# p768lwy3/torecsys

Measured on AMD Instinct MI355X. Metric: CTR samples/sec fwd+bwd (DeepFM, 39 fields x dim 64), higher is better.
Workload: dtype bf16; 1 GPU; BASELINE.json configs[1]: DeepFM 39 Criteo-shaped fields, MLP [400,400,400], 1000000 total rows, embed_dim 64, batch 65536, uniform indices, uniform field sizes; global_batch=65536, rows=1000000, parallelism=single, microbatches=1, optimizer=none, hipgraph=True, hipgraph_input_sets=1, hipgraph_steps_per_replay=4, fused_lookup_fm=True

## Files before the change

### include/trs_abi.h

```cpp
#ifndef TRS_ABI_H_
#define TRS_ABI_H_

#include <stddef.h>
#include <stdint.h>

#ifdef __cplusplus
extern "C" {
#endif

#define TRS_ABI_VERSION 3

enum { TRS_F32 = 0, TRS_BF16 = 1 };
enum { TRS_I64 = 0, TRS_I32 = 1 };
enum {
  TRS_OK = 0,
  TRS_EINVAL = -1,
  TRS_EDTYPE = -2,
  TRS_ESHAPE = -3,
  TRS_EALIGN = -4,
  TRS_ELAUNCH = -5,
  TRS_EWORKSPACE = -6
};

typedef void* trs_stream_t;
// ... 184 lines not shown
int trs_rowdot_fwd(const void* h, const void* w, const void* bias, int64_t rows, int32_t C, int32_t dtype, void* out,
                   trs_stream_t stream);
size_t trs_rowdot_bwd_workspace_bytes(int64_t rows, int32_t C);
int trs_rowdot_bwd(const void* g, const void* h, const void* w, int64_t rows, int32_t C, int32_t dtype, void* gh,
                   float* gw, float* gb, void* workspace, size_t ws_bytes, trs_stream_t stream);

int trs_transpose_pad(const void* in, int64_t B, int32_t R, int32_t Cc, int32_t ld_in, void* out, int32_t ld_out,
                      int32_t dtype, trs_stream_t stream);

int trs_cat_head_fwd(const void* a, const void* d, const void* w, const void* bias, int64_t rows, int32_t N, int32_t Ea,
                     int32_t Eb, int32_t dtype, void* out, trs_stream_t stream);
size_t trs_cat_head_bwd_workspace_bytes(int64_t rows, int32_t N, int32_t Ea, int32_t Eb);
int trs_cat_head_bwd(const void* g, const void* a, const void* d, const void* w, int64_t rows, int32_t N, int32_t Ea,
                     int32_t Eb, int32_t dtype, void* ga, void* gd, float* gw, float* gb, void* workspace,
                     size_t ws_bytes, trs_stream_t stream);

int trs_wgrad_finish(const float* part, int32_t S, int32_t R, int32_t Cc, int32_t out_rows, int32_t out_cols,
                     int32_t dtype, void* gw, const float* gb_f32, void* gb, trs_stream_t stream);
int trs_wgrad_finish_t(const float* part, int32_t S, int32_t Cc, int32_t R, int32_t out_rows, int32_t out_cols,
                       int32_t dtype, void* gw, const float* gb_f32, void* gb, trs_stream_t stream);
int32_t trs_wgrad_rows_splits(int32_t M, int32_t N, int64_t rows);
int trs_wgrad_rows(const void* g, int32_t ldg, const void* x, int32_t ldx, int64_t rows, int32_t M, int32_t N,
                   int32_t dtype, int32_t S, float* part, trs_stream_t stream);
int32_t trs_wgrad_wide_splits(int32_t M_x, int32_t N_g, int32_t ld_g, int64_t rows);
int trs_wgrad_wide(const void* x, int32_t ldx, const void* g, int32_t ldg, int64_t rows, int32_t M_x, int32_t N_g,
                   int32_t S, float* part, trs_stream_t stream);
int trs_copy_padded_many(const int64_t* desc, int32_t n, int32_t elem_size, int64_t max_elems, trs_stream_t stream);

int32_t trs_cin_glue_blocks(int64_t B);
int trs_cin_glue_stats(const void* y, int64_t B, int32_t E, int32_t C, int32_t dtype, float* partial,
                       trs_stream_t stream);
int trs_cin_glue_fwd(const void* y, const float* scale, const float* shift, int64_t B, int32_t E, int32_t C, int32_t D,
                     int32_t Hs, int32_t dtype, void* hidden, void* pooled, trs_stream_t stream);
int trs_cin_glue_bwd_reduce(const void* y, const void* g_hidden, const void* g_pooled, const float* scale,
                            const float* shift, const float* mean, const float* invstd, int64_t B, int32_t E, int32_t C,
                            int32_t D, int32_t Hs, int32_t dtype, float* partial, trs_stream_t stream);
int trs_cin_glue_bwd_apply(const void* y, const void* g_hidden, const void* g_pooled, const float* scale,
                           const float* shift, const float* mean, const float* invstd, const float* c1, const float* c2,
                           int64_t B, int32_t E, int32_t C, int32_t D, int32_t Hs, int32_t dtype, void* gy,
                           trs_stream_t stream);
int trs_cin_glue_cf_supported(int32_t E, int32_t C);
int trs_cin_glue_fwd_cf(const void* y, const float* scale, const float* shift, int64_t B, int32_t E, int32_t C,
                        int32_t D, int32_t Hs, int32_t dtype, void* hidden, void* hidden_cf, void* pooled,
                        trs_stream_t stream);
int trs_cin_glue_bwd_apply_cf(const void* y, const void* g_hidden, const void* g_pooled, const float* scale,
                              const float* shift, const float* mean, const float* invstd, const float* c1,
// ... 124 lines not shown
```

### torecsys_amd/_abi.py

```python
from __future__ import annotations

import ctypes
import os
import threading
from ctypes import c_char_p, c_int32, c_int64, c_size_t, c_void_p

import torch

_HERE = os.path.dirname(os.path.abspath(__file__))
LIB_PATH = os.environ.get("TRS_LIB_PATH") or os.path.join(_HERE, "libtrs_hip.so")

TRS_F32, TRS_BF16 = 0, 1
TRS_I64, TRS_I32 = 0, 1

_P, _I32, _I64, _SZ, _F32 = c_void_p, c_int32, c_int64, c_size_t, ctypes.c_float

_OPTIMIZER_TAIL = [_I32, _F32, _P, _F32, _F32, _F32, _P, _P, _P, _SZ, _P]

SIGNATURES = {
    "trs_version": (c_int32, []),
    "trs_last_error_string": (c_char_p, []),
    "trs_rowdot_fwd": (c_int32, [_P, _P, _P, _I64, _I32, _I32, _P, _P]),
    "trs_rowdot_bwd_workspace_bytes": (_SZ, [_I64, _I32]),
    "trs_rowdot_bwd": (c_int32, [_P, _P, _P, _I64, _I32, _I32, _P, _P, _P, _P, _SZ, _P]),
    "trs_transpose_pad": (c_int32, [_P, _I64, _I32, _I32, _I32, _P, _I32, _I32, _P]),
    "trs_cat_head_fwd": (c_int32, [_P, _P, _P, _P, _I64, _I32, _I32, _I32, _I32, _P, _P]),
    "trs_cat_head_bwd_workspace_bytes": (_SZ, [_I64, _I32, _I32, _I32]),
    "trs_cat_head_bwd": (c_int32, [_P, _P, _P, _P, _I64, _I32, _I32, _I32, _I32, _P, _P, _P, _P, _P, _SZ, _P]),
    "trs_wgrad_finish": (c_int32, [_P, _I32, _I32, _I32, _I32, _I32, _I32, _P, _P, _P, _P]),
    "trs_wgrad_finish_t": (c_int32, [_P, _I32, _I32, _I32, _I32, _I32, _I32, _P, _P, _P, _P]),
    "trs_wgrad_rows_splits": (c_int32, [_I32, _I32, _I64]),
    "trs_wgrad_rows": (c_int32, [_P, _I32, _P, _I32, _I64, _I32, _I32, _I32, _I32, _P, _P]),
    "trs_wgrad_wide_splits": (c_int32, [_I32, _I32, _I32, _I64]),
    "trs_wgrad_wide": (c_int32, [_P, _I32, _P, _I32, _I64, _I32, _I32, _I32, _P, _P]),
    "trs_copy_padded_many": (c_int32, [_P, _I32, _I32, _I64, _P]),
    "trs_cin_glue_blocks": (c_int32, [_I64]),
    "trs_cin_glue_stats": (c_int32, [_P, _I64, _I32, _I32, _I32, _P, _P]),
    "trs_cin_glue_fwd": (c_int32, [_P, _P, _P, _I64, _I32, _I32, _I32, _I32, _I32, _P, _P, _P]),
    "trs_cin_glue_bwd_reduce": (c_int32, [_P, _P, _P, _P, _P, _P, _P, _I64, _I32, _I32, _I32, _I32, _I32, _P, _P]),
    "trs_cin_glue_bwd_apply": (c_int32, [_P, _P, _P, _P, _P, _P, _P, _P, _P, _I64, _I32, _I32, _I32, _I32, _I32, _P, _P]),
    "trs_cin_glue_cf_supported": (c_int32, [_I32, _I32]),
    "trs_cin_glue_fwd_cf": (c_int32, [_P, _P, _P, _I64, _I32, _I32, _I32, _I32, _I32, _P, _P, _P, _P]),
    "trs_cin_glue_bwd_apply_cf": (c_int32, [_P, _P, _P, _P, _P, _P, _P, _P, _P, _I64, _I32, _I32, _I32, _I32, _I32, _P, _P, _P,
                                            _P]),
    "trs_opn_vec_fwd": (c_int32, [_P, _P, _I32, _I64, _I32, _I32, _I32, _P, _P]),
    "trs_opn_vec_bwd_workspace_bytes": (_SZ, [_I64, _I32, _I32]),
    "trs_opn_vec_bwd": (c_int32, [_P, _P, _P, _I32, _I64, _I32, _I32, _I32, _P, _P, _P, _SZ, _P]),
    "trs_pair_mul_fwd": (c_int32, [_P, _P, _P, _I32, _I64, _I32, _I32, _I32, _P, _P]),
    "trs_rows_mul_bias_fwd": (c_int32, [_P, _P, _P, _I32, _I64, _I32, _I32, _I32, _P, _P]),
    "trs_rows_mul_bwd": (c_int32, [_P, _P, _P, _I64, _I32, _I32, _P, _P, _P]),
    "trs_pair_mul_bwd": (c_int32, [_P, _P, _P, _I64, _I32, _I32, _I32, _P, _P, _P]),
    "trs_pair_bilinear_fwd": (c_int32, [_P, _P, _I32, _P, _I32, _I32, _I64, _I32, _I32, _I32, _P, _P]),
    "trs_pair_bilinear_bwd_data": (c_int32, [_P, _P, _P, _I32, _I32, _I64, _I32, _I32, _I32, _P, _P, _P]),
    "trs_pair_bilinear_fwd_mfma": (c_int32, [_P, _P, _P, _P, _I32, _I32, _I64, _I32, _I32, _I32, _P, _P]),
    "trs_pair_bilinear_bwd_data_mfma": (c_int32, [_P, _P, _P, _P, _P, _I32, _P, _P, _I32, _P, _I32, _I64, _I32, _I32, _I32,
# ... 319 lines not shown
```

### torecsys_amd/csrc/mlp_epilogue.hip

```cpp
#include <algorithm>

#include "trs_common.hpp"

namespace trs {

constexpr int RB_THREADS = 256;

template <typename T>
__global__ __launch_bounds__(RB_THREADS) void relu_bwd_bias_kernel(const uint4* __restrict__ gy, const uint4* __restrict__ y,
                                                                   uint4* __restrict__ gz, float* __restrict__ part,
                                                                   int64_t rows, int vpr ,
                                                                   int rows_per_band) {
  constexpr int VE = Vec16<T>::VE;
  __shared__ float red[RB_THREADS][VE];
  const int64_t r0 = (int64_t)blockIdx.x * rows_per_band;
  const int64_t r1 = r0 + rows_per_band < rows ? r0 + rows_per_band : rows;
  const int cv = threadIdx.x % vpr, rl = threadIdx.x / vpr, rstep = RB_THREADS / vpr;
  float acc[VE];
#pragma unroll
  for (int k = 0; k < VE; ++k) acc[k] = 0.f;
  if (rl < rstep) {
    constexpr int U = 4;
    for (int64_t rb = r0 + rl; rb < r1; rb += (int64_t)rstep * U) {
      uint4 gv[U], yv[U];
// ... 188 lines not shown

__global__ void rowdot_finish_kernel(const float* __restrict__ tmp, int C, float* __restrict__ gw,
                                         float* __restrict__ gb) {
  const int c = blockIdx.x * blockDim.x + threadIdx.x;
  if (c < C) gw[c] = tmp[c];
  else if (c == C) gb[0] = tmp[C];
}

static int rowdot_fwd_blocks(int64_t rows, int lpr) {
  const int rpp = 256 / lpr;
  return (int)std::min<int64_t>((rows + (int64_t)rpp * 4 - 1) / ((int64_t)rpp * 4), 8192);
}
static int rowdot_blocks(int64_t rows, int lpr) {
  const int rpp = 256 / lpr;
  return (int)std::min<int64_t>((rows + rpp - 1) / rpp, 1023);
}
static bool rowdot_shape_ok(int C, int dtype) {
  const int ve = dtype == TRS_F32 ? 4 : 8;
  const int lpr = C % ve == 0 ? C / ve : 0;
  return lpr >= 1 && lpr <= 64 && (lpr & (lpr - 1)) == 0;
}

template <typename T>
__global__ __launch_bounds__(256) void wgrad_finish_kernel(const float* __restrict__ part, int S, int R, int Cc,
                                                          int out_rows, int out_cols, T* __restrict__ gw,
                                                          const float* __restrict__ gbf, T* __restrict__ gb) {
  const int c = blockIdx.x * 256 + threadIdx.x;
  if ((int)blockIdx.y == out_rows) {
    if (gb != nullptr && c < out_rows) gb[c] = from_f32<T>(gbf[c]);
    return;
  }
  if (c >= out_cols) return;
  const int r = blockIdx.y;
  const float* p = part + (size_t)r * Cc + c;
  const size_t stride = (size_t)R * Cc;
  float a0 = 0.f, a1 = 0.f, a2 = 0.f, a3 = 0.f;
  int s = 0;
  for (; s + 4 <= S; s += 4) {
    a0 += p[(size_t)s * stride];
    a1 += p[(size_t)(s + 1) * stride];
    a2 += p[(size_t)(s + 2) * stride];
    a3 += p[(size_t)(s + 3) * stride];
  }
  for (; s < S; ++s) a0 += p[(size_t)s * stride];
  gw[(size_t)r * out_cols + c] = from_f32<T>((a0 + a1) + (a2 + a3));
}

constexpr int WF_SL = 16;
constexpr int WF_COLS = 256 / WF_SL;
template <typename T>
__global__ __launch_bounds__(256) void wgrad_finish_few_rows_kernel(const float* __restrict__ part, int S, int R, int Cc,
                                                                   int out_rows, int out_cols, T* __restrict__ gw,
                                                                   const float* __restrict__ gbf, T* __restrict__ gb) {
  __shared__ float red[WF_SL][WF_COLS + 1];
  if ((int)blockIdx.y == out_rows) {
    const int c = blockIdx.x * 256 + threadIdx.x;
    if (gb != nullptr && c < out_rows) gb[c] = from_f32<T>(gbf[c]);
    return;
  }
  const int cl = threadIdx.x % WF_COLS, sl = threadIdx.x / WF_COLS;
  const int c = blockIdx.x * WF_COLS + cl;
  const int r = blockIdx.y;
  const size_t stride = (size_t)R * Cc;
  float a0 = 0.f, a1 = 0.f, a2 = 0.f, a3 = 0.f;
  if (c < out_cols) {
    const float* p = part + (size_t)r * Cc + c;
    int s = sl;
    for (; s + 3 * WF_SL < S; s += 4 * WF_SL) {
// ... 382 lines not shown
  TRS_REQUIRE(gb == nullptr || out_rows <= ((out_cols + 255) / 256) * 256, TRS_ESHAPE,
              "wgrad_finish: out_rows %d exceeds the bias row of workgroups", out_rows);
  hipStream_t s = (hipStream_t)stream;
  dim3 grid((out_cols + 255) / 256, out_rows + 1);
  if (S >= 4 * WF_SL && (int64_t)grid.x * out_rows < 64) {
    dim3 gridf((out_cols + WF_COLS - 1) / WF_COLS, out_rows + 1);
    if (dtype == TRS_F32)
      hipLaunchKernelGGL((wgrad_finish_few_rows_kernel<float>), gridf, dim3(256), 0, s, part, S, R, Cc, out_rows, out_cols,
                         (float*)gw, gb_f32, (float*)gb);
    else
      hipLaunchKernelGGL((wgrad_finish_few_rows_kernel<bf16_t>), gridf, dim3(256), 0, s, part, S, R, Cc, out_rows, out_cols,
                         (bf16_t*)gw, gb_f32, (bf16_t*)gb);
    return check_launch("wgrad_finish");
  }
  if (dtype == TRS_F32)
    hipLaunchKernelGGL((wgrad_finish_kernel<float>), grid, dim3(256), 0, s, part, S, R, Cc, out_rows, out_cols,
                       (float*)gw, gb_f32, (float*)gb);
  else
    hipLaunchKernelGGL((wgrad_finish_kernel<bf16_t>), grid, dim3(256), 0, s, part, S, R, Cc, out_rows, out_cols,
                       (bf16_t*)gw, gb_f32, (bf16_t*)gb);
  return check_launch("wgrad_finish");
}

extern "C" int trs_wgrad_finish_t(const float* part, int32_t S, int32_t Cc, int32_t R, int32_t out_rows, int32_t out_cols,
                                  int32_t dtype, void* gw, const float* gb_f32, void* gb, trs_stream_t stream) {
  TRS_REQUIRE(S > 0 && R > 0 && Cc > 0 && out_rows > 0 && out_cols > 0 && out_rows <= R && out_cols <= Cc, TRS_EINVAL,
              "wgrad_finish_t: bad size");
  TRS_REQUIRE(part && gw, TRS_EINVAL, "wgrad_finish_t: NULL pointer");
  TRS_REQUIRE((gb == nullptr) == (gb_f32 == nullptr), TRS_EINVAL, "wgrad_finish_t: gb and gb_f32 go together");
  TRS_REQUIRE(dtype == TRS_F32 || dtype == TRS_BF16, TRS_EDTYPE, "wgrad_finish_t: dtype %d", dtype);
  hipStream_t s = (hipStream_t)stream;
  dim3 grid((out_rows + 31) / 32, (out_cols + 31) / 32 + 1);
  if (dtype == TRS_F32)
    hipLaunchKernelGGL((wgrad_finish_t_kernel<float>), grid, dim3(256), 0, s, part, S, Cc, R, out_rows, out_cols,
                       (float*)gw, gb_f32, (float*)gb);
  else
    hipLaunchKernelGGL((wgrad_finish_t_kernel<bf16_t>), grid, dim3(256), 0, s, part, S, Cc, R, out_rows, out_cols,
                       (bf16_t*)gw, gb_f32, (bf16_t*)gb);
  return check_launch("wgrad_finish_t");
}

namespace trs {
__global__ __launch_bounds__(256) void copy_padded_many_kernel(const int64_t* __restrict__ desc, int elem_size) {
  const int64_t* d = desc + (size_t)blockIdx.y * 6;
  const char* src = reinterpret_cast<const char*>(d[0]);
  char* dst = reinterpret_cast<char*>(d[1]);
// ... 57 lines not shown
```

### torecsys_amd/csrc/wgrad_rows.hip

```cpp
#include <algorithm>

#include "trs_common.hpp"

namespace trs {

typedef __attribute__((ext_vector_type(4))) short wg_s16x4;
typedef __attribute__((ext_vector_type(8))) short wg_s16x8;
typedef __attribute__((ext_vector_type(8))) __bf16 wg_bf16x8;
typedef __attribute__((ext_vector_type(4))) float wg_f32x4;

constexpr int WG_KR = 64;
constexpr int WG_KS = 32;
constexpr int WG_PANEL = WG_KS * 32 + 32;
constexpr int WG_TC = 7;

struct WgradArgs {
  const uint16_t* g;
  const uint16_t* x;
  float* part;
  int64_t rows;
  int ldg, ldx;
  int M, N;
  int MB, NB;
  int slots_per_xcd;
  int S;
};

__host__ __device__ __forceinline__ int split_start(int total, int parts, int k) { return (int)(((int64_t)total * k) / parts); }

__device__ __forceinline__ wg_bf16x8 tr_frag(const char* lo_p, const char* hi_p, int off) {
  typedef __attribute__((address_space(3))) wg_s16x4* lds_p;
  const wg_s16x4 lo = __builtin_amdgcn_ds_read_tr16_b64_v4i16((lds_p)(lo_p + off));
  const wg_s16x4 hi = __builtin_amdgcn_ds_read_tr16_b64_v4i16((lds_p)(hi_p + off));
  const wg_s16x8 v = {lo[0], lo[1], lo[2], lo[3], hi[0], hi[1], hi[2], hi[3]};
  return __builtin_bit_cast(wg_bf16x8, v);
}

__device__ __forceinline__ void wg_mfma(wg_f32x4& acc, const wg_bf16x8& A, const wg_bf16x8& B) {
  asm volatile("v_mfma_f32_16x16x32_bf16 %0, %1, %2, %0" : "+a"(acc) : "v"(A), "v"(B));
}

template <int WM, int WN, int MC, int NC, bool CHECK>
__global__ __launch_bounds__(64 * WM * WN, 1) void wgrad_rows_kernel(WgradArgs a) {
  constexpr int NWAVES = WM * WN;
  constexpr bool EXACT = NWAVES == 8;
  extern __shared__ __attribute__((aligned(16))) char wg_lds[];
  const int lane = threadIdx.x & 63, wave = __builtin_amdgcn_readfirstlane(threadIdx.x >> 6);
  const int q = lane >> 4, i = lane & 15;
  const bool odd = q & 1;

  const int TB = a.MB * a.NB;
// ... 143 lines not shown
    run.template operator()<MC, NC>();
  } else {
    if (mc == MC && nc == NC) run.template operator()<MC, NC>();
    else if (mc == MC) run.template operator()<MC, NC - 1>();
    else if (nc == NC) run.template operator()<MC - 1, NC>();
    else run.template operator()<MC - 1, NC - 1>();
  }
}

constexpr int WD_S = 416;
constexpr int WD_IMG = WG_KS * WD_S;
constexpr int WD_SLOT = 2 * WD_IMG;
constexpr int WD_NSLOT = 6;
constexpr int WD_AHEAD = 5;

__device__ __forceinline__ void wd_dma(const char* src, unsigned voff, unsigned lds_dst) {
  unsigned keep;
  const unsigned dst = __builtin_amdgcn_readfirstlane(lds_dst);
  asm volatile("s_mov_b32 %0, m0\n\ts_mov_b32 m0, %2\n\ts_nop 0\n\tglobal_load_lds_dwordx4 %1, %3\n\ts_mov_b32 m0, %0"
               : "=&s"(keep) : "v"(voff), "s"(dst), "s"(src) : "memory");
}

template <int MC, int NC>
__global__ __launch_bounds__(512, 1) void wgrad_dma_kernel(WgradArgs a) {
  extern __shared__ __attribute__((aligned(16))) char wg_lds[];
  const int lane = threadIdx.x & 63, wave = __builtin_amdgcn_readfirstlane(threadIdx.x >> 6);
  const int q = lane >> 4, i = lane & 15;
  const bool odd = q & 1;
  const int TB = a.MB * a.NB;
  const int xcd = blockIdx.x & 7, j = blockIdx.x >> 3;
  const int slot = xcd * a.slots_per_xcd + j / TB;
  const int S = 8 * a.slots_per_xcd;
  const int tile = j % TB;
  const int mb = tile / a.NB, nb = tile % a.NB;
  const int Mt = (a.M + 15) >> 4, Nt = (a.N + 15) >> 4;
  const int bm0 = split_start(Mt, a.MB, mb), bm1 = split_start(Mt, a.MB, mb + 1);
  const int bn0 = split_start(Nt, a.NB, nb), bn1 = split_start(Nt, a.NB, nb + 1);
  const int PM = bm1 - bm0, PN = bn1 - bn0;
  const int wm = wave >> 2, wn = wave >= 4 ? ((wave + 1) & 3) : (wave & 3);
  const int am0 = split_start(PM, 2, wm), mc = split_start(PM, 2, wm + 1) - am0;
  const int an0 = split_start(PN, 4, wn), nc = split_start(PN, 4, wn + 1) - an0;
  const int64_t quads_total = a.rows / (4 * WG_KS);
  const int64_t h0 = 4 * (quads_total * slot / S), h1 = 4 * (quads_total * (slot + 1) / S);
  const int64_t n_h = h1 - h0;

  const char* gcol = reinterpret_cast<const char*>(a.g + 16 * bm0);
  const char* xcol = reinterpret_cast<const char*>(a.x + 16 * bn0);
  unsigned voff[4];
#pragma unroll
  for (int t = 0; t < 4; ++t) {
    const int p = wave + 8 * t, op = p >= 13, jj = op ? p - 13 : p;
    const int o = jj * 1024 + 16 * lane, row = o / WD_S, cb = o - row * WD_S;
    voff[t] = (unsigned)(row * (op ? a.ldx : a.ldg) * 2 + cb);
  }
  const unsigned lds0 = (unsigned)(uintptr_t)(__attribute__((address_space(3))) const char*)wg_lds;
  auto issue = [&](int64_t k, unsigned ring_slot) __attribute__((always_inline)) {
// ... 251 lines not shown
    } else if (pm_lo >= 12 && pm_hi <= 14 && pn_lo >= 8 && pn_hi <= 12) {
      p.wn = 4;
      p.mc = 7;
      p.nc = 3;
    }
  }
  auto blocks_ok = [](int T, int B, int cols) {
    for (int b = 0; b < B; ++b) {
      const int t0 = split_start(T, B, b), t1 = split_start(T, B, b + 1);
      if (t1 - t0 < 12 || t1 - t0 > 13 || 16 * t0 + 208 > cols) return false;
    }
    return true;
  };
  if (p.wm == 2 && p.wn == 4 && p.nc == 4 && rows % (4 * WG_KS) == 0 && blocks_ok(Mt, p.MB, M) &&
      blocks_ok(Nt, p.NB, N))
    p.dma = (p.NB == 2 && rows >= WD2_MIN_ROWS) ? 2 : 1;
  int slots = 32 / (p.dma == 2 ? p.MB : p.MB * p.NB);
  const int64_t stages = (rows + WG_KR - 1) / WG_KR;
  while (slots > 1 && stages / (8 * slots) < 4) slots >>= 1;
  p.slots_per_xcd = slots;
  return p;
}

template <int WM, int WN, int MC, int NC, bool CHECK>
int wgrad_launch_c(const WgradArgs& a, int grid, size_t lds, hipStream_t s) {
  static bool attr = false;
  if (!attr) {
    if (hipFuncSetAttribute((const void*)wgrad_rows_kernel<WM, WN, MC, NC, CHECK>, hipFuncAttributeMaxDynamicSharedMemorySize,
                            160 * 1024) != hipSuccess)
      return check_launch("wgrad_rows: LDS attribute");
    attr = true;
  }
  hipLaunchKernelGGL((wgrad_rows_kernel<WM, WN, MC, NC, CHECK>), dim3(grid), dim3(64 * WM * WN), lds, s, a);
  return check_launch("wgrad_rows");
}

}

using namespace trs;

template <int WM, int WN, int MC, int NC>
static int wgrad_launch(const WgradArgs& a, int grid, size_t lds, hipStream_t s) {
  return (a.rows % (4 * WG_KS)) ? wgrad_launch_c<WM, WN, MC, NC, true>(a, grid, lds, s)
                          : wgrad_launch_c<WM, WN, MC, NC, false>(a, grid, lds, s);
}

static int wgrad_dma2_launch(const WgradArgs& a, int grid, hipStream_t s, const char* what) {
  static bool attr2 = false;
  if (!attr2) {
    if (hipFuncSetAttribute((const void*)wgrad_dma2_kernel, hipFuncAttributeMaxDynamicSharedMemorySize, 160 * 1024) != hipSuccess)
      return check_launch("wgrad_dma2: LDS attribute");
    attr2 = true;
  }
  hipLaunchKernelGGL(wgrad_dma2_kernel, dim3(grid), dim3(256), (size_t)WD2_NSLOT * WD2_SLOT, s, a);
  return check_launch(what);
}

extern "C" int32_t trs_wgrad_rows_splits(int32_t M, int32_t N, int64_t rows) {
  const WgradPlan p = wgrad_plan(M, N, rows);
  return 8 * p.slots_per_xcd;
}

extern "C" int trs_wgrad_rows(const void* g, int32_t ldg, const void* x, int32_t ldx, int64_t rows, int32_t M, int32_t N,
                              int32_t dtype, int32_t S, float* part, trs_stream_t stream) {
  TRS_REQUIRE(dtype == TRS_BF16, TRS_EDTYPE, "wgrad_rows: bf16 operands only");
  WgradPlan p = wgrad_plan(M, N, rows);
  TRS_REQUIRE(p.slots_per_xcd > 0 && S == 8 * p.slots_per_xcd, TRS_ESHAPE,
              "wgrad_rows: (M=%d, N=%d, rows=%lld) takes %d row ranges, caller passed %d", M, N, (long long)rows,
              8 * p.slots_per_xcd, S);
  TRS_REQUIRE(ldg >= M && ldx >= N && (ldg & 7) == 0 && (ldx & 7) == 0 && aligned16(g) && aligned16(x), TRS_ESHAPE,
              "wgrad_rows: row strides must be multiples of 8 elements and cover M / N, operands 16-byte aligned");
  if (!g || !x || !part) return fail(TRS_EINVAL, "wgrad_rows: null pointer");
  hipStream_t s = (hipStream_t)stream;
  WgradArgs a{(const uint16_t*)g, (const uint16_t*)x, part, rows, ldg, ldx, M, N, p.MB, p.NB, p.slots_per_xcd, 0};
  const int Mt = (M + 15) / 16, Nt = (N + 15) / 16;
  const int PM = (Mt + p.MB - 1) / p.MB, PN = (Nt + p.NB - 1) / p.NB;
  const size_t lds = (size_t)(4 * (PM + PN) + WG_TC) * WG_PANEL;
  const int grid = 8 * p.slots_per_xcd * p.MB * p.NB;
  TRS_REQUIRE(p.dma == 0 || (int64_t)WG_KS * std::max(ldg, ldx) * 2 < ((int64_t)1 << 31), TRS_ESHAPE, "wgrad_rows: row stride too large");
  if (p.dma == 2) {
    a.S = 8 * p.slots_per_xcd;
    return wgrad_dma2_launch(a, a.S * p.MB, s, "wgrad_rows(dma2)");
  }
  if (p.dma == 1) {
    static bool attr = false;
    if (!attr) {
      if (hipFuncSetAttribute((const void*)wgrad_dma_kernel<7, 4>, hipFuncAttributeMaxDynamicSharedMemorySize, 160 * 1024) != hipSuccess)
        return check_launch("wgrad_rows(dma): LDS attribute");
      attr = true;
    }
    hipLaunchKernelGGL((wgrad_dma_kernel<7, 4>), dim3(grid), dim3(512), (size_t)WD_NSLOT * WD_SLOT, s, a);
    return check_launch("wgrad_rows(dma)");
  }
  if (p.wm == 2 && p.wn == 4)
    return p.nc == 4 ? wgrad_launch<2, 4, 7, 4>(a, grid, lds, s) : wgrad_launch<2, 4, 7, 3>(a, grid, lds, s);
  if (p.wm == 2)
    return p.nc == 5 ? wgrad_launch<2, 2, WG_TC, 5>(a, grid, lds, s) : wgrad_launch<2, 2, WG_TC, WG_TC>(a, grid, lds, s);
  if (p.wm == 4) return p.nc == 4 ? wgrad_launch<4, 1, WG_TC, 4>(a, grid, lds, s) : wgrad_launch<4, 1, WG_TC, WG_TC>(a, grid, lds, s);
  if (p.mc == 1) return wgrad_launch<1, 4, 1, WG_TC>(a, grid, lds, s);
  if (p.mc == 4) return wgrad_launch<1, 4, 4, WG_TC>(a, grid, lds, s);
  return wgrad_launch<1, 4, WG_TC, WG_TC>(a, grid, lds, s);
}

struct WidePlan {
  int spx, S, grid;
};

static WidePlan wide_plan(int MB) {
  WidePlan w{std::min(32 / MB, 4), 0, 0};
  const int extra = w.spx == 32 / MB ? 8 * (32 - w.spx * MB) / MB : 0;
  w.S = 8 * w.spx + extra;
  w.grid = 8 * (w.spx * MB + (extra * MB + 7) / 8);
  return w;
}

extern "C" int32_t trs_wgrad_wide_splits(int32_t M_x, int32_t N_g, int32_t ld_g, int64_t rows) {
  if (M_x < 2 * 208 || M_x % 208 || N_g < 8 || (N_g & 15) || (ld_g & 7) || rows <= 0 || rows % (4 * WG_KS)) return 0;
  const int Nt = N_g / 16, MB = M_x / 208;
  if (Nt < 24 || Nt > 26 || 16 * split_start(Nt, 2, 1) + 208 > ld_g || MB > 32) return 0;
  if ((int64_t)WG_KS * std::max(M_x, ld_g) * 2 >= ((int64_t)1 << 31)) return 0;
  const int S = wide_plan(MB).S;
  return rows >= (int64_t)4 * WG_KS * S ? S : 0;
}

// ... 14 lines not shown
```

### torecsys_amd/functional.py

```python
from __future__ import annotations

import ctypes
import os
from typing import List, Optional, Sequence, Tuple

import torch
from torch.autograd import Function
from torch.autograd.function import once_differentiable

from . import _abi
from ._abi import call, index_dtype_code, ptr, require_device, size_query, stream_ptr, value_dtype_code

CHECK_INDICES = os.environ.get("TRS_CHECK_INDICES", "0") not in ("", "0")


def _as_index(idx: torch.Tensor) -> torch.Tensor:
    idx = idx.rename(None) if idx.has_names() else idx
    if idx.dtype not in (torch.int64, torch.int32):
        if idx.dtype.is_floating_point or idx.dtype == torch.bool:
            raise TypeError(f"indices must be an integer tensor, got {idx.dtype}")
        idx = idx.long()
    return idx.contiguous()


# ... 2530 lines not shown
    def forward(ctx, x, *params):
        require_device(x, *params)
        L = len(params) // 2
        Ws = [params[2 * l].contiguous() for l in range(L)]
        bs = [params[2 * l + 1].contiguous() for l in range(L)]
        widths = [Ws[0].shape[1]] + [w.shape[0] for w in Ws]
        x2 = x.reshape(-1, widths[0]).contiguous()
        y, hidden, masks, fam = fused_mlp_forward_raw(x2, Ws, bs)
        ctx.save_for_backward(x2, *Ws, *hidden, *masks)
        ctx.meta = (L, widths, tuple(x.shape), [p.dtype for p in params], fam)
        return y.reshape(*x.shape[:-1], widths[L])

    @staticmethod
    @once_differentiable
    def backward(ctx, gy):
        L, widths, xshape, pdt, fam = ctx.meta
        saved = ctx.saved_tensors
        x2, Ws = saved[0], saved[1:1 + L]
        hidden, masks = saved[1 + L:L + L], saved[L + L:]
        rows, dev = x2.shape[0], x2.device
        gy2 = gy.reshape(rows, widths[L]).contiguous()
        gx, gz, gb, _ = fused_mlp_backward_raw(gy2, widths, Ws, masks, family=fam)
        grads = []
        for l in range(L):
            inp = x2 if l == 0 else hidden[l - 1]
            g = gy2 if l == L - 1 else gz[l]
            need_w, need_b = ctx.needs_input_grad[1 + 2 * l], ctx.needs_input_grad[2 + 2 * l]
            if pdt[2 * l] == pdt[2 * l + 1]:
                gw, gbias = _tail_layer_grads(g, inp, widths[l + 1], widths[l], pdt[2 * l], gb[l], need_w, need_b)
            else:
                gw = _wgrad_rows(g, inp, widths[l + 1], widths[l], pdt[2 * l]) if need_w else None
                gbias = gb[l][:widths[l + 1]].to(pdt[2 * l + 1]) if need_b else None
            grads += [gw, gbias]
        return (gx.reshape(xshape) if ctx.needs_input_grad[0] else None, *grads)


ROWS_GEMM = os.environ.get("TRS_ROWS_GEMM", "1") not in ("", "0")
ROWS_GEMM_MIN_COLS = 1024


def rows_gemm_supported_for(rows: int, x_stride: int, W: torch.Tensor, out_f: int, in_f: int) -> bool:
    if not (ROWS_GEMM and W.is_cuda and W.dtype == torch.bfloat16 and W.is_contiguous() and rows >= 4096
            and in_f >= ROWS_GEMM_MIN_COLS and W.shape[1] == in_f and W.shape[0] >= out_f):
        return False
    return bool(_abi.load().trs_rows_gemm_supported(int(out_f), int(in_f), int(x_stride)))


def rows_gemm_supported(g: torch.Tensor, W: torch.Tensor, out_f: int, in_f: int) -> bool:
    if not (g.is_cuda and g.dtype == torch.bfloat16 and g.dim() == 2 and g.is_contiguous()):
        return False
    return rows_gemm_supported_for(g.shape[0], g.shape[1], W, out_f, in_f)


def rows_gemm(g: torch.Tensor, W: torch.Tensor, out_f: int, in_f: int) -> torch.Tensor:
    y = torch.empty(g.shape[0], in_f, dtype=torch.bfloat16, device=g.device)
    ws_bytes = size_query("trs_rows_gemm_workspace_bytes", out_f, in_f)
    ws = torch.empty(ws_bytes, dtype=torch.uint8, device=g.device)
    call("trs_rows_gemm", ptr(g), g.shape[0], g.shape[1], ptr(W), out_f, in_f, _abi.TRS_BF16, ptr(y), ptr(ws), ws_bytes,
         stream_ptr())
    return y


def _tail_layer_grads(g, inp, out_f, in_f, dtype, gb_f32, need_w, need_b):
    if need_w and need_b:
        return _wgrad_rows(g, inp, out_f, in_f, dtype, gb_f32)
    gw = _wgrad_rows(g, inp, out_f, in_f, dtype) if need_w else None
    return gw, (gb_f32[:out_f].to(dtype) if need_b else None)


WGRAD_ROWS = os.environ.get("TRS_WGRAD_ROWS", "1") not in ("", "0")


def pad_cols(g: torch.Tensor, width: int) -> torch.Tensor:
    g = g.contiguous()
    out = torch.empty(g.shape[0], width, dtype=g.dtype, device=g.device)
    call("trs_pad_cols", ptr(g), g.shape[1], ptr(out), width, g.shape[0], value_dtype_code(g), stream_ptr())
    return out


def _wgrad_rows(g: torch.Tensor, inp: torch.Tensor, out_f: int, in_f: int, dtype, gb_f32: Optional[torch.Tensor] = None):
    if gb_f32 is not None:
        gb = torch.empty(out_f, dtype=dtype, device=g.device)
        if out_f <= (in_f + 255) // 256 * 256:
            return _wgrad_rows_impl(g, inp, out_f, in_f, dtype, gb_f32, gb), gb
        gb.copy_(gb_f32[:out_f])
        return _wgrad_rows_impl(g, inp, out_f, in_f, dtype, None, None), gb
    return _wgrad_rows_impl(g, inp, out_f, in_f, dtype, None, None)


def _wgrad_rows_impl(g, inp, out_f, in_f, dtype, gb_f32, gb):
# ... 117 lines not shown
```

### torecsys_amd/layers.py

```python
from __future__ import annotations

from abc import ABC, abstractmethod
from typing import Dict, List, Optional, Tuple

import math
import os

import torch
import torch.nn as nn

from . import functional as F_


def _strip(t: torch.Tensor) -> torch.Tensor:
    return t.rename(None) if t.has_names() else t


class BaseLayer(nn.Module, ABC):

    def __init__(self, **kwargs):
        super().__init__()

    @property
    @abstractmethod
# ... 717 lines not shown
                                                                      family=F_.MLP_FAMILY_MIXED, x_stride=h1.shape[1])
        else:
            y, hidden, masks, mask_in, fam = F_.fused_mlp_forward_raw(h1, Ws, bs, input_mask=True)
        out_f = tail[4 * (L - 1)].shape[0]
        ctx.save_for_backward(cur, W1, h1, mask_in, *Ws, *hidden, *masks)
        ctx.meta = (L, [h1.shape[1]] + [w.shape[0] for w in Ws], [tuple(tail[4 * l].shape) for l in range(L)],
                    [tail[4 * l].dtype for l in range(L)], tuple(w1.shape), w1.dtype, tuple(x.shape), fam)
        y = y[:, :out_f] if out_f != y.shape[1] else y
        return y.reshape(*x.shape[:-1], out_f)

    @staticmethod
    @torch.autograd.function.once_differentiable
    def backward(ctx, gy):
        L, widths, wshapes, wdt, w1shape, w1dt, xshape, fam = ctx.meta
        saved = ctx.saved_tensors
        cur, W1, h1, mask_in = saved[:4]
        Ws = saved[4:4 + L]
        hidden, masks = saved[4 + L:3 + L + L], saved[3 + L + L:]
        needs = ctx.needs_input_grad
        gy = gy.reshape(h1.shape[0], -1)
        gy2 = F_.pad_cols(gy, widths[L]) if gy.shape[1] != widths[L] else gy.contiguous()
        g1, gz, gb, gb1 = F_.fused_mlp_backward_raw(gy2, widths, Ws, masks, mask_in, family=fam)
        grads = []
        for l in range(L):
            inp = h1 if l == 0 else hidden[l - 1]
            g = gy2 if l == L - 1 else gz[l]
            out_f, in_f = wshapes[l]
            grads += [*F_._tail_layer_grads(g, inp, out_f, in_f, wdt[l], gb[l], needs[6 + 4 * l], needs[7 + 4 * l]),
                      None, None]
        gx, gw1, gbias1 = _dense_layer_grads(g1, gb1, cur, W1, w1shape[0], w1shape[1], w1dt, needs[0], needs[2], needs[3])
        return (gx.reshape(xshape) if needs[0] else None, None, gw1, gbias1, None, None, *grads)


class _MLPStack(torch.autograd.Function):

    SPLIT_ROWS_WIDE = 4096

    @staticmethod
    def forward(ctx, x, spec, *tensors):
        cur = x.reshape(-1, x.shape[-1])
        saved, wmeta = [], []
        for l, (fuse, rowdot) in enumerate(spec):
            weight, bias, w_use, b_use = tensors[4 * l:4 * l + 4]
            W = weight if w_use is None else w_use
            Bv = bias if w_use is None else b_use
            if rowdot:
                Wf = W.reshape(-1)
                out = torch.empty(cur.shape[0], 1, dtype=cur.dtype, device=cur.device)
                F_.call("trs_rowdot_fwd", F_.ptr(cur), F_.ptr(Wf), F_.ptr(Bv), cur.shape[0], cur.shape[1],
                        F_.value_dtype_code(cur), F_.ptr(out), F_.stream_ptr())
                W = Wf
            elif fuse:
# ... 376 lines not shown
```

Before: 59.44 million samples/s.

## Batch MLP tail-layer weight-gradient GEMMs and finishes into grouped launches

Adds grouped variants of the DMA row-split weight-gradient kernel and the split-reduction finish kernel, so several hidden layers' wgrad jobs run in one launch with blocks mapped across jobs and XCDs. The MLP backward paths now collect the tail layers (all but the last) into a batch and issue one grouped wgrad launch and one grouped finish launch. The goal is to cut per-layer launch overhead and fill the GPU better when each individual wgrad is too small to occupy it. In exchange, each job gets fewer row splits (slots divided by the job count), and the path only applies when all jobs share the same tile plan.

Result: faster. 60.54 million samples/s, median of 6 (+1.8%).

```diff
diff --git a/include/trs_abi.h b/include/trs_abi.h
--- a/include/trs_abi.h
+++ b/include/trs_abi.h
@@ -230,6 +230,16 @@
 int32_t trs_wgrad_rows_splits(int32_t M, int32_t N, int64_t rows);
 int trs_wgrad_rows(const void* g, int32_t ldg, const void* x, int32_t ldx, int64_t rows, int32_t M, int32_t N,
                    int32_t dtype, int32_t S, float* part, trs_stream_t stream);
+int32_t trs_wgrad_rows_many_splits(int32_t n_jobs, const int32_t* M, const int32_t* N, const int32_t* ldg,
+                                   const int32_t* ldx, int64_t rows);
+int32_t trs_wgrad_rows_many_map(int32_t n_jobs, const int32_t* M, const int32_t* N, const int32_t* ldg,
+                                const int32_t* ldx, int64_t rows, int32_t block, int64_t* out);
+int trs_wgrad_rows_many(int32_t n_jobs, const void* const* g, const int32_t* ldg, const void* const* x,
+                        const int32_t* ldx, int64_t rows, const int32_t* M, const int32_t* N, int32_t S,
+                        float* const* part, trs_stream_t stream);
+int trs_wgrad_finish_many(int32_t n_jobs, const float* const* part, int32_t S, const int32_t* R, const int32_t* Cc,
+                          const int32_t* out_rows, const int32_t* out_cols, int32_t dtype, void* const* gw,
+                          const float* const* gb_f32, void* const* gb, trs_stream_t stream);
 int32_t trs_wgrad_wide_splits(int32_t M_x, int32_t N_g, int32_t ld_g, int64_t rows);
 int trs_wgrad_wide(const void* x, int32_t ldx, const void* g, int32_t ldg, int64_t rows, int32_t M_x, int32_t N_g,
                    int32_t S, float* part, trs_stream_t stream);
diff --git a/torecsys_amd/_abi.py b/torecsys_amd/_abi.py
--- a/torecsys_amd/_abi.py
+++ b/torecsys_amd/_abi.py
@@ -31,6 +31,10 @@
     "trs_wgrad_finish_t": (c_int32, [_P, _I32, _I32, _I32, _I32, _I32, _I32, _P, _P, _P, _P]),
     "trs_wgrad_rows_splits": (c_int32, [_I32, _I32, _I64]),
     "trs_wgrad_rows": (c_int32, [_P, _I32, _P, _I32, _I64, _I32, _I32, _I32, _I32, _P, _P]),
+    "trs_wgrad_rows_many_splits": (c_int32, [_I32, _P, _P, _P, _P, _I64]),
+    "trs_wgrad_rows_many_map": (c_int32, [_I32, _P, _P, _P, _P, _I64, _I32, _P]),
+    "trs_wgrad_rows_many": (c_int32, [_I32, _P, _P, _P, _P, _I64, _P, _P, _I32, _P, _P]),
+    "trs_wgrad_finish_many": (c_int32, [_I32, _P, _I32, _P, _P, _P, _P, _I32, _P, _P, _P, _P]),
     "trs_wgrad_wide_splits": (c_int32, [_I32, _I32, _I32, _I64]),
     "trs_wgrad_wide": (c_int32, [_P, _I32, _P, _I32, _I64, _I32, _I32, _I32, _P, _P]),
     "trs_copy_padded_many": (c_int32, [_P, _I32, _I32, _I64, _P]),
diff --git a/torecsys_amd/csrc/mlp_epilogue.hip b/torecsys_amd/csrc/mlp_epilogue.hip
--- a/torecsys_amd/csrc/mlp_epilogue.hip
+++ b/torecsys_amd/csrc/mlp_epilogue.hip
@@ -234,15 +234,15 @@
 }
 
 template <typename T>
-__global__ __launch_bounds__(256) void wgrad_finish_kernel(const float* __restrict__ part, int S, int R, int Cc,
-                                                          int out_rows, int out_cols, T* __restrict__ gw,
-                                                          const float* __restrict__ gbf, T* __restrict__ gb) {
+__device__ __forceinline__ void wgrad_finish_body(const float* __restrict__ part, int S, int R, int Cc, int out_rows,
+                                                  int out_cols, T* __restrict__ gw, const float* __restrict__ gbf,
+                                                  T* __restrict__ gb) {
   const int c = blockIdx.x * 256 + threadIdx.x;
   if ((int)blockIdx.y == out_rows) {
     if (gb != nullptr && c < out_rows) gb[c] = from_f32<T>(gbf[c]);
     return;
   }
-  if (c >= out_cols) return;
+  if ((int)blockIdx.y > out_rows || c >= out_cols) return;
   const int r = blockIdx.y;
   const float* p = part + (size_t)r * Cc + c;
   const size_t stride = (size_t)R * Cc;
@@ -256,6 +256,31 @@
   }
   for (; s < S; ++s) a0 += p[(size_t)s * stride];
   gw[(size_t)r * out_cols + c] = from_f32<T>((a0 + a1) + (a2 + a3));
+}
+
+template <typename T>
+__global__ __launch_bounds__(256) void wgrad_finish_kernel(const float* __restrict__ part, int S, int R, int Cc,
+                                                          int out_rows, int out_cols, T* __restrict__ gw,
+                                                          const float* __restrict__ gbf, T* __restrict__ gb) {
+  wgrad_finish_body<T>(part, S, R, Cc, out_rows, out_cols, gw, gbf, gb);
+}
+
+constexpr int WF_MAXJ = 8;
+struct WgradFinishJob {
+  const float* part;
+  void* gw;
+  const float* gbf;
+  void* gb;
+  int R, Cc, out_rows, out_cols;
+};
+struct WgradFinishArgs {
+  WgradFinishJob job[WF_MAXJ];
+  int S;
+};
+template <typename T>
+__global__ __launch_bounds__(256) void wgrad_finish_many_kernel(WgradFinishArgs a) {
+  const WgradFinishJob& j = a.job[blockIdx.z];
+  wgrad_finish_body<T>(j.part, a.S, j.R, j.Cc, j.out_rows, j.out_cols, (T*)j.gw, j.gbf, (T*)j.gb);
 }
 
 constexpr int WF_SL = 16;
@@ -684,6 +709,35 @@
   return check_launch("wgrad_finish");
 }
 
+extern "C" int trs_wgrad_finish_many(int32_t n_jobs, const float* const* part, int32_t S, const int32_t* R,
+                                     const int32_t* Cc, const int32_t* out_rows, const int32_t* out_cols, int32_t dtype,
+                                     void* const* gw, const float* const* gb_f32, void* const* gb, trs_stream_t stream) {
+  TRS_REQUIRE(n_jobs >= 1 && n_jobs <= WF_MAXJ, TRS_EINVAL, "wgrad_finish_many: %d jobs (1 .. %d)", n_jobs, WF_MAXJ);
+  TRS_REQUIRE(part && R && Cc && out_rows && out_cols && gw && gb_f32 && gb, TRS_EINVAL, "wgrad_finish_many: NULL array");
+  TRS_REQUIRE(S > 0, TRS_EINVAL, "wgrad_finish_many: bad size");
+  TRS_REQUIRE(dtype == TRS_F32 || dtype == TRS_BF16, TRS_EDTYPE, "wgrad_finish_many: dtype %d", dtype);
+  WgradFinishArgs a{};
+  a.S = S;
+  int max_rows = 0, max_cols = 0;
+  for (int k = 0; k < n_jobs; ++k) {
+    TRS_REQUIRE(R[k] > 0 && Cc[k] > 0 && out_rows[k] > 0 && out_cols[k] > 0 && out_rows[k] <= R[k] && out_cols[k] <= Cc[k],
+                TRS_EINVAL, "wgrad_finish_many: bad size (job %d)", k);
+    TRS_REQUIRE(part[k] && gw[k], TRS_EINVAL, "wgrad_finish_many: NULL pointer (job %d)", k);
+    TRS_REQUIRE((gb[k] == nullptr) == (gb_f32[k] == nullptr), TRS_EINVAL, "wgrad_finish_many: gb and gb_f32 go together (job %d)", k);
+    TRS_REQUIRE(gb[k] == nullptr || out_rows[k] <= ((out_cols[k] + 255) / 256) * 256, TRS_ESHAPE,
+                "wgrad_finish_many: out_rows %d exceeds the bias row of workgroups", out_rows[k]);
+    a.job[k] = WgradFinishJob{part[k], gw[k], gb_f32[k], gb[k], R[k], Cc[k], out_rows[k], out_cols[k]};
+    max_rows = std::max(max_rows, out_rows[k]);
+    max_cols = std::max(max_cols, out_cols[k]);
+  }
+  dim3 grid((max_cols + 255) / 256, max_rows + 1, n_jobs);
+  if (dtype == TRS_F32)
+    hipLaunchKernelGGL((wgrad_finish_many_kernel<float>), grid, dim3(256), 0, (hipStream_t)stream, a);
+  else
+    hipLaunchKernelGGL((wgrad_finish_many_kernel<bf16_t>), grid, dim3(256), 0, (hipStream_t)stream, a);
+  return check_launch("wgrad_finish_many");
+}
+
 extern "C" int trs_wgrad_finish_t(const float* part, int32_t S, int32_t Cc, int32_t R, int32_t out_rows, int32_t out_cols,
                                   int32_t dtype, void* gw, const float* gb_f32, void* gb, trs_stream_t stream) {
   TRS_REQUIRE(S > 0 && R > 0 && Cc > 0 && out_rows > 0 && out_cols > 0 && out_rows <= R && out_cols <= Cc, TRS_EINVAL,
diff --git a/torecsys_amd/csrc/wgrad_rows.hip b/torecsys_amd/csrc/wgrad_rows.hip
--- a/torecsys_amd/csrc/wgrad_rows.hip
+++ b/torecsys_amd/csrc/wgrad_rows.hip
@@ -27,6 +27,27 @@
 };
 
 __host__ __device__ __forceinline__ int split_start(int total, int parts, int k) { return (int)(((int64_t)total * k) / parts); }
+
+constexpr int WG_MAXJ = 8;
+struct WgradJob {
+  const uint16_t* g;
+  const uint16_t* x;
+  float* part;
+  int ldg, ldx, M, N;
+};
+struct WgradManyArgs {
+  WgradJob job[WG_MAXJ];
+  int64_t rows;
+  int J, MB, NB, slots_per_xcd;
+};
+
+__host__ __device__ __forceinline__ void wdm_place(int TB, int spx, int b, int& job, int& slot, int& tile) {
+  const int xcd = b & 7, j = b >> 3, per_job = spx * TB;
+  job = j / per_job;
+  const int r = j - job * per_job;
+  slot = xcd * spx + r / TB;
+  tile = r % TB;
+}
 
 __device__ __forceinline__ wg_bf16x8 tr_frag(const char* lo_p, const char* hi_p, int off) {
   typedef __attribute__((address_space(3))) wg_s16x4* lds_p;
@@ -216,16 +237,16 @@
 }
 
 template <int MC, int NC>
-__global__ __launch_bounds__(512, 1) void wgrad_dma_kernel(WgradArgs a) {
+__global__ __launch_bounds__(512, 1) void wgrad_dma_kernel(WgradManyArgs am) {
   extern __shared__ __attribute__((aligned(16))) char wg_lds[];
   const int lane = threadIdx.x & 63, wave = __builtin_amdgcn_readfirstlane(threadIdx.x >> 6);
   const int q = lane >> 4, i = lane & 15;
   const bool odd = q & 1;
-  const int TB = a.MB * a.NB;
-  const int xcd = blockIdx.x & 7, j = blockIdx.x >> 3;
-  const int slot = xcd * a.slots_per_xcd + j / TB;
+  int jb, slot, tile;
+  wdm_place(am.MB * am.NB, am.slots_per_xcd, blockIdx.x, jb, slot, tile);
+  const WgradJob& jd = am.job[jb];
+  const WgradArgs a{jd.g, jd.x, jd.part, am.rows, jd.ldg, jd.ldx, jd.M, jd.N, am.MB, am.NB, am.slots_per_xcd, 0};
   const int S = 8 * a.slots_per_xcd;
-  const int tile = j % TB;
   const int mb = tile / a.NB, nb = tile % a.NB;
   const int Mt = (a.M + 15) >> 4, Nt = (a.N + 15) >> 4;
   const int bm0 = split_start(Mt, a.MB, mb), bm1 = split_start(Mt, a.MB, mb + 1);
@@ -523,6 +544,30 @@
   return p;
 }
 
+struct ManyPlan {
+  int S = 0, MB = 0, NB = 0, slots_per_xcd = 0, grid = 0;
+};
+
+static ManyPlan wgrad_many_plan(int J, const int32_t* M, const int32_t* N, const int32_t* ldg, const int32_t* ldx, int64_t rows) {
+  ManyPlan mp;
+  if (J < 1 || J > WG_MAXJ || !M || !N || !ldg || !ldx || rows <= 0) return mp;
+  int MB = 0, NB = 0;
+  for (int k = 0; k < J; ++k) {
+    if (ldg[k] < M[k] || ldx[k] < N[k] || (ldg[k] & 7) || (ldx[k] & 7)) return mp;
+    if ((int64_t)WG_KS * std::max(ldg[k], ldx[k]) * 2 >= ((int64_t)1 << 31)) return mp;
+    const WgradPlan p = wgrad_plan(M[k], N[k], rows);
+    if (p.slots_per_xcd == 0 || p.dma != 1) return mp;
+    if (k > 0 && (p.MB != MB || p.NB != NB)) return mp;
+    MB = p.MB, NB = p.NB;
+    const int Mt = (M[k] + 15) / 16, Nt = (N[k] + 15) / 16;
+    if (16 * split_start(Mt, MB, MB - 1) + 208 > ldg[k] || 16 * split_start(Nt, NB, NB - 1) + 208 > ldx[k]) return mp;
+  }
+  const int spx = 32 / (MB * NB * J);
+  if (spx < 1 || rows / WG_KR / (8 * spx) < 4) return mp;
+  mp.S = 8 * spx, mp.MB = MB, mp.NB = NB, mp.slots_per_xcd = spx, mp.grid = 8 * spx * MB * NB * J;
+  return mp;
+}
+
 template <int WM, int WN, int MC, int NC, bool CHECK>
 int wgrad_launch_c(const WgradArgs& a, int grid, size_t lds, hipStream_t s) {
   static bool attr = false;
@@ -554,6 +599,17 @@
     attr2 = true;
   }
   hipLaunchKernelGGL(wgrad_dma2_kernel, dim3(grid), dim3(256), (size_t)WD2_NSLOT * WD2_SLOT, s, a);
+  return check_launch(what);
+}
+
+static int wgrad_dma_launch(const WgradManyArgs& am, int grid, hipStream_t s, const char* what) {
+  static bool attr = false;
+  if (!attr) {
+    if (hipFuncSetAttribute((const void*)wgrad_dma_kernel<7, 4>, hipFuncAttributeMaxDynamicSharedMemorySize, 160 * 1024) != hipSuccess)
+      return check_launch("wgrad_rows(dma): LDS attribute");
+    attr = true;
+  }
+  hipLaunchKernelGGL((wgrad_dma_kernel<7, 4>), dim3(grid), dim3(512), (size_t)WD_NSLOT * WD_SLOT, s, am);
   return check_launch(what);
 }
 
@@ -584,14 +640,10 @@
     return wgrad_dma2_launch(a, a.S * p.MB, s, "wgrad_rows(dma2)");
   }
   if (p.dma == 1) {
-    static bool attr = false;
-    if (!attr) {
-      if (hipFuncSetAttribute((const void*)wgrad_dma_kernel<7, 4>, hipFuncAttributeMaxDynamicSharedMemorySize, 160 * 1024) != hipSuccess)
-        return check_launch("wgrad_rows(dma): LDS attribute");
-      attr = true;
-    }
-    hipLaunchKernelGGL((wgrad_dma_kernel<7, 4>), dim3(grid), dim3(512), (size_t)WD_NSLOT * WD_SLOT, s, a);
-    return check_launch("wgrad_rows(dma)");
+    WgradManyArgs am{};
+    am.job[0] = WgradJob{a.g, a.x, part, ldg, ldx, M, N};
+    am.rows = rows, am.J = 1, am.MB = p.MB, am.NB = p.NB, am.slots_per_xcd = p.slots_per_xcd;
+    return wgrad_dma_launch(am, grid, s, "wgrad_rows(dma)");
   }
   if (p.wm == 2 && p.wn == 4)
     return p.nc == 4 ? wgrad_launch<2, 4, 7, 4>(a, grid, lds, s) : wgrad_launch<2, 4, 7, 3>(a, grid, lds, s);
@@ -601,6 +653,42 @@
   if (p.mc == 1) return wgrad_launch<1, 4, 1, WG_TC>(a, grid, lds, s);
   if (p.mc == 4) return wgrad_launch<1, 4, 4, WG_TC>(a, grid, lds, s);
   return wgrad_launch<1, 4, WG_TC, WG_TC>(a, grid, lds, s);
+}
+
+extern "C" int32_t trs_wgrad_rows_many_splits(int32_t n_jobs, const int32_t* M, const int32_t* N, const int32_t* ldg,
+                                              const int32_t* ldx, int64_t rows) {
+  return wgrad_many_plan(n_jobs, M, N, ldg, ldx, rows).S;
+}
+
+extern "C" int32_t trs_wgrad_rows_many_map(int32_t n_jobs, const int32_t* M, const int32_t* N, const int32_t* ldg,
+                                           const int32_t* ldx, int64_t rows, int32_t block, int64_t* out) {
+  const ManyPlan mp = wgrad_many_plan(n_jobs, M, N, ldg, ldx, rows);
+  if (mp.S == 0 || !out || block < 0 || block >= mp.grid) return 0;
+  int job, slot, tile;
+  wdm_place(mp.MB * mp.NB, mp.slots_per_xcd, block, job, slot, tile);
+  const int64_t quads = rows / (4 * WG_KS);
+  out[0] = job, out[1] = slot, out[2] = tile;
+  out[3] = 4 * WG_KS * (quads * slot / mp.S), out[4] = 4 * WG_KS * (quads * (slot + 1) / mp.S);
+  return mp.grid;
+}
+
+extern "C" int trs_wgrad_rows_many(int32_t n_jobs, const void* const* g, const int32_t* ldg, const void* const* x,
+                                   const int32_t* ldx, int64_t rows, const int32_t* M, const int32_t* N, int32_t S,
+                                   float* const* part, trs_stream_t stream) {
+  TRS_REQUIRE(n_jobs >= 1 && n_jobs <= WG_MAXJ, TRS_EINVAL, "wgrad_rows_many: %d jobs (1 .. %d)", n_jobs, WG_MAXJ);
+  if (!g || !x || !part || !ldg || !ldx || !M || !N) return fail(TRS_EINVAL, "wgrad_rows_many: null pointer");
+  const ManyPlan mp = wgrad_many_plan(n_jobs, M, N, ldg, ldx, rows);
+  TRS_REQUIRE(mp.S > 0 && S == mp.S, TRS_ESHAPE, "wgrad_rows_many: %d jobs over %lld rows take %d row ranges each, caller passed %d",
+              n_jobs, (long long)rows, mp.S, S);
+  WgradManyArgs am{};
+  for (int k = 0; k < n_jobs; ++k) {
+    if (!g[k] || !x[k] || !part[k]) return fail(TRS_EINVAL, "wgrad_rows_many: null pointer (job %d)", k);
+    TRS_REQUIRE(aligned16(g[k]) && aligned16(x[k]) && aligned16(part[k]), TRS_ESHAPE,
+                "wgrad_rows_many: operands of job %d not 16-byte aligned", k);
+    am.job[k] = WgradJob{(const uint16_t*)g[k], (const uint16_t*)x[k], part[k], ldg[k], ldx[k], M[k], N[k]};
+  }
+  am.rows = rows, am.J = n_jobs, am.MB = mp.MB, am.NB = mp.NB, am.slots_per_xcd = mp.slots_per_xcd;
+  return wgrad_dma_launch(am, mp.grid, (hipStream_t)stream, "wgrad_rows_many");
 }
 
 struct WidePlan {
diff --git a/torecsys_amd/functional.py b/torecsys_amd/functional.py
--- a/torecsys_amd/functional.py
+++ b/torecsys_amd/functional.py
@@ -2576,6 +2576,12 @@
         gy2 = gy.reshape(rows, widths[L]).contiguous()
         gx, gz, gb, _ = fused_mlp_backward_raw(gy2, widths, Ws, masks, family=fam)
         grads = []
+        if all(pdt[2 * l] == pdt[2 * l + 1] for l in range(L)):
+            for gw, gbias in _tail_grads([(gy2 if l == L - 1 else gz[l], x2 if l == 0 else hidden[l - 1], widths[l + 1],
+                                           widths[l], pdt[2 * l], gb[l], ctx.needs_input_grad[1 + 2 * l],
+                                           ctx.needs_input_grad[2 + 2 * l]) for l in range(L)]):
+                grads += [gw, gbias]
+            return (gx.reshape(xshape) if ctx.needs_input_grad[0] else None, *grads)
         for l in range(L):
             inp = x2 if l == 0 else hidden[l - 1]
             g = gy2 if l == L - 1 else gz[l]
@@ -2620,6 +2626,52 @@
         return _wgrad_rows(g, inp, out_f, in_f, dtype, gb_f32)
     gw = _wgrad_rows(g, inp, out_f, in_f, dtype) if need_w else None
     return gw, (gb_f32[:out_f].to(dtype) if need_b else None)
+
+
+def _wgrad_many_splits(jobs) -> int:
+    if not WGRAD_ROWS or len(jobs) < 2:
+        return 0
+    for g, inp, _, _ in jobs:
+        if not (g.is_cuda and g.dtype == torch.bfloat16 and inp.dtype == torch.bfloat16 and g.is_contiguous()
+                and inp.is_contiguous() and g.shape[0] == jobs[0][0].shape[0]):
+            return 0
+    return size_query("trs_wgrad_rows_many_splits", len(jobs), _i32_array([j[2] for j in jobs]),
+                      _i32_array([j[3] for j in jobs]), _i32_array([j[0].shape[1] for j in jobs]),
+                      _i32_array([j[1].shape[1] for j in jobs]), int(jobs[0][0].shape[0]))
+
+
+def _tail_grads(layers):
+    out = [None] * len(layers)
+    batch = [k for k, t in enumerate(layers[:-1]) if t[6]]
+    jobs = [(layers[k][0], layers[k][1], min(layers[k][0].shape[1], (layers[k][2] + 7) // 8 * 8),
+             min(layers[k][1].shape[1], (layers[k][3] + 7) // 8 * 8)) for k in batch]
+    S = _wgrad_many_splits(jobs) if len({layers[k][4] for k in batch}) == 1 else 0
+    if S > 0:
+        dev, dtype, rows = jobs[0][0].device, layers[batch[0]][4], jobs[0][0].shape[0]
+        parts = [torch.empty(S, M, N, dtype=torch.float32, device=dev) for _, _, M, N in jobs]
+        call("trs_wgrad_rows_many", len(jobs), _ptr_array([j[0] for j in jobs]), _i32_array([j[0].shape[1] for j in jobs]),
+             _ptr_array([j[1] for j in jobs]), _i32_array([j[1].shape[1] for j in jobs]), rows,
+             _i32_array([j[2] for j in jobs]), _i32_array([j[3] for j in jobs]), S, _ptr_array(parts), stream_ptr())
+        gws, gbs, gbfs = [], [], []
+        for k in batch:
+            _, _, out_f, in_f, _, gb_f32, _, need_b = layers[k]
+            gws.append(torch.empty(out_f, in_f, dtype=dtype, device=dev))
+            ride = need_b and out_f <= (in_f + 255) // 256 * 256
+            gbs.append(torch.empty(out_f, dtype=dtype, device=dev) if ride else None)
+            gbfs.append(gb_f32 if ride else None)
+        call("trs_wgrad_finish_many", len(jobs), _ptr_array(parts), S, _i32_array([j[2] for j in jobs]),
+             _i32_array([j[3] for j in jobs]), _i32_array([layers[k][2] for k in batch]),
+             _i32_array([layers[k][3] for k in batch]), value_dtype_code(gws[0]), _ptr_array(gws), _ptr_array(gbfs),
+             _ptr_array(gbs), stream_ptr())
+        for n, k in enumerate(batch):
+            gb = gbs[n]
+            if gb is None and layers[k][7]:
+                gb = layers[k][5][:layers[k][2]].to(dtype)
+            out[k] = (gws[n], gb)
+    for k, t in enumerate(layers):
+        if out[k] is None:
+            out[k] = _tail_layer_grads(*t)
+    return out
 
 
 WGRAD_ROWS = os.environ.get("TRS_WGRAD_ROWS", "1") not in ("", "0")
diff --git a/torecsys_amd/layers.py b/torecsys_amd/layers.py
--- a/torecsys_amd/layers.py
+++ b/torecsys_amd/layers.py
@@ -763,12 +763,9 @@
         gy2 = F_.pad_cols(gy, widths[L]) if gy.shape[1] != widths[L] else gy.contiguous()
         g1, gz, gb, gb1 = F_.fused_mlp_backward_raw(gy2, widths, Ws, masks, mask_in, family=fam)
         grads = []
-        for l in range(L):
-            inp = h1 if l == 0 else hidden[l - 1]
-            g = gy2 if l == L - 1 else gz[l]
-            out_f, in_f = wshapes[l]
-            grads += [*F_._tail_layer_grads(g, inp, out_f, in_f, wdt[l], gb[l], needs[6 + 4 * l], needs[7 + 4 * l]),
-                      None, None]
+        for gw, gbias in F_._tail_grads([(gy2 if l == L - 1 else gz[l], h1 if l == 0 else hidden[l - 1], *wshapes[l],
+                                          wdt[l], gb[l], needs[6 + 4 * l], needs[7 + 4 * l]) for l in range(L)]):
+            grads += [gw, gbias, None, None]
         gx, gw1, gbias1 = _dense_layer_grads(g1, gb1, cur, W1, w1shape[0], w1shape[1], w1dt, needs[0], needs[2], needs[3])
         return (gx.reshape(xshape) if needs[0] else None, None, gw1, gbias1, None, None, *grads)
 
```
